# Jamy-L/Handheld-Multi-Frame-Super-Resolution

Hardware: AMD Instinct MI355X
Metric: output Mpix/s for 12MP x 20-frame x2 SR burst; max-abs diff vs reference (higher is better)
Workload: dtype f32

## Files before the change

### handheld-multi-frame-super-resolution_amd/csrc/hhsr_fft.hip

```cpp
#include "hhsr_common.h"
#include "hhsr_fft.h"
#include <math.h>
#include <type_traits>
#include <vector>

#include "hhsr_fft_bfly.h"

__host__ __device__ constexpr int fft_maxit(int R) { return R <= 3 ? 4 : R <= 5 ? 3 : R <= 12 ? 2 : 1; }

template <int R>
__device__ __forceinline__ void stockham_pass(float2* __restrict__ buf, int bstride, int NB,
                                              const float2* __restrict__ twp, int N, int Ns, int tid, int nt, bool pw) {
    constexpr int MAXIT = fft_maxit(R);
    const int L = N / R, total = NB * L;
    const float rNs = 1.0f / (float)Ns, rL = 1.0f / (float)L;
    float2 v[MAXIT][R];
    int dst[MAXIT];
#pragma unroll
    for (int it = 0; it < MAXIT; ++it) {
        const int jj = tid + it * nt;
        if (jj < total) {
            const int bidx = NB > 1 ? (int)(((float)jj + 0.5f) * rL) : 0;
            const int j = jj - __mul24(bidx, L);
            const int q = (int)(((float)j + 0.5f) * rNs);
            const int k = j - __mul24(q, Ns);
            const int base = __mul24(bidx, bstride);
            const float2* ib = buf + base + j;
#pragma unroll
            for (int r = 0; r < R; ++r) v[it][r] = ib[__mul24(r, L)];
            if (Ns > 1) {
                if (R <= HHSR_FFT_POW_RMAX && pw) {
                    float2 w[R];
                    w[1] = twp[k];
#pragma unroll
                    for (int r = 2; r < R; ++r) w[r] = cmul(w[r >> 1], w[r - (r >> 1)]);
#pragma unroll
                    for (int r = 1; r < R; ++r) v[it][r] = cmul(v[it][r], w[r]);
                } else {
#pragma unroll
                    for (int r = 1; r < R; ++r) v[it][r] = cmul(v[it][r], twp[__mul24(r - 1, Ns) + k]);
                }
            }
            dft_reg<R>(v[it]);
            dst[it] = base + __mul24(q * R, Ns) + k;
        }
    }
    __syncthreads();
#pragma unroll
    for (int it = 0; it < MAXIT; ++it) {
        const int jj = tid + it * nt;
        if (jj < total) {
#pragma unroll
            for (int r = 0; r < R; ++r) buf[dst[it] + __mul24(r, Ns)] = v[it][r];
        }
    }
    __syncthreads();
}

template <bool PR>
__device__ __forceinline__ void fft_lds(float2* buf, int bstride, int NB, const float2* tw, int N,
                                        const HhsrRadices& rad, int tid, int nt) {
    int Ns = 1, toff = 0;
    __syncthreads();
    for (int p = 0; p < rad.n; ++p) {
        const int R = rad.r[p];
        int Np = N;
        asm volatile("" : "+s"(Np));
        const bool pw = rad.pow_min > 0 && R <= HHSR_FFT_POW_RMAX && (R - 1) * Ns > rad.pow_min;
        switch (R) {
#define HHSR_PASS(RR) case RR: stockham_pass<RR>(buf, bstride, NB, tw + toff, Np, Ns, tid, nt, pw); break;
            HHSR_PASS(2) HHSR_PASS(3) HHSR_PASS(4) HHSR_PASS(5) HHSR_PASS(6) HHSR_PASS(7) HHSR_PASS(8) HHSR_PASS(9)
            HHSR_PASS(10) HHSR_PASS(12) HHSR_PASS(14) HHSR_PASS(15) HHSR_PASS(16)
            default:
                if constexpr (PR) {
                    switch (R) {
                        HHSR_PASS(11) HHSR_PASS(13) HHSR_PASS(17) HHSR_PASS(19)
                        default: break;
                    }
                }
                break;
#undef HHSR_PASS
        }
        toff += pw ? Ns : (R - 1) * Ns;
        Ns *= R;
    }
}

template <int N_, int... RS>
struct SPlan {
    static constexpr int N = N_;
    static constexpr int NP = (int)sizeof...(RS);
    static constexpr int R[NP] = {RS...};
    static constexpr int ns(int p) {
        int s = 1;
        for (int i = 0; i < p; ++i) s *= R[i];
        return s;
    }
    static constexpr bool pw(int p) {
        return HHSR_FFT_POW_MIN > 0 && R[p] <= HHSR_FFT_POW_RMAX && (R[p] - 1) * ns(p) > HHSR_FFT_POW_MIN;
    }
    static constexpr int toff(int p) {
        int o = 0;
        for (int i = 0; i < p; ++i) o += pw(i) ? ns(i) : (R[i] - 1) * ns(i);
        return o;
    }
    static constexpr int rmax() {
        int m = 0;
        for (int i = 0; i < NP; ++i) m = R[i] > m ? R[i] : m;
        return m;
    }
    static bool matches(int n, const HhsrRadices& rad) {
        if (n != N || rad.n != NP || rad.pow_min != HHSR_FFT_POW_MIN) return false;
        for (int i = 0; i < NP; ++i)
            if (rad.r[i] != R[i]) return false;
        return true;
    }
};
struct NoPlan {
    static constexpr int N = 0;
    static constexpr int rmax() { return 16; }
};
struct PrimePlan {
    static constexpr int N = 0;
    static constexpr int rmax() { return 19; }
};
template <class SP>
constexpr bool plan_runtime = std::is_same<SP, NoPlan>::value || std::is_same<SP, PrimePlan>::value;
template <class SP>
__device__ __forceinline__ int plan_len(int runtime) {
    return plan_runtime<SP> ? runtime : SP::N;
}

template <int N, int NB, int NT, int R, int Ns, bool PW>
__device__ __forceinline__ void stockham_pass_s(float2* __restrict__ buf, const float2* __restrict__ twp, int tid) {
    constexpr int MAXIT = fft_maxit(R), L = N / R, total = NB * L;
    float2 v[MAXIT][R];
    int dst[MAXIT];
#pragma unroll
    for (int it = 0; it < MAXIT; ++it) {
        const int jj = tid + it * NT;
        if (it * NT < total && jj < total) {
            const int bidx = NB > 1 ? (int)((unsigned)jj / (unsigned)L) : 0;
            const int j = jj - bidx * L;
            const int q = (int)((unsigned)j / (unsigned)Ns), k = j - q * Ns;
            const float2* ib = buf + bidx * N + j;
#pragma unroll
            for (int r = 0; r < R; ++r) v[it][r] = ib[r * L];
            if (Ns > 1) {
                if (R <= HHSR_FFT_POW_RMAX && PW) {
                    float2 w[R];
                    w[1] = twp[k];
#pragma unroll
                    for (int r = 2; r < R; ++r) w[r] = cmul(w[r >> 1], w[r - (r >> 1)]);
#pragma unroll
                    for (int r = 1; r < R; ++r) v[it][r] = cmul(v[it][r], w[r]);
                } else {
#pragma unroll
                    for (int r = 1; r < R; ++r) v[it][r] = cmul(v[it][r], twp[(r - 1) * Ns + k]);
                }
            }
            dft_reg<R>(v[it]);
            dst[it] = bidx * N + q * (R * Ns) + k;
        }
    }
    __syncthreads();
#pragma unroll
    for (int it = 0; it < MAXIT; ++it) {
        const int jj = tid + it * NT;
        if (it * NT < total && jj < total) {
#pragma unroll
            for (int r = 0; r < R; ++r) buf[dst[it] + r * Ns] = v[it][r];
        }
    }
    __syncthreads();
}

template <class P, int NB, int NT, int PASS = 0>
__device__ __forceinline__ void fft_lds_s(float2* buf, const float2* tw, int tid) {
    if (PASS == 0) __syncthreads();
    if constexpr (PASS < P::NP) {
        stockham_pass_s<P::N, NB, NT, P::R[PASS], P::ns(PASS), P::pw(PASS)>(buf, tw + P::toff(PASS), tid);
        fft_lds_s<P, NB, NT, PASS + 1>(buf, tw, tid);
    }
}

#define HHSR_STATIC_ROWS(X)                                                                 \
    X(1, 2000, 1, FFT_NT_SMALL, 10, 10, 10, 2)              \
    X(2, 4000, 1, FFT_NT, 10, 10, 10, 4)                        \
    X(3, 2016, 1, FFT_NT_SMALL, 14, 12, 12)     \
    X(4, 2040, 1, FFT_NT_SMALL, 17, 15, 8)      \
    X(5, 2736, 2, FFT_NT, 19, 16, 9)
#define HHSR_STATIC_COLS(X)                                                                 \
    X(1, 3000, 2, FFT_NT, 3, 10, 10, 10)                             \
    X(2, 6000, 1, FFT_NT, 10, 10, 10, 6)                             \
    X(3, 3024, 2, FFT_NT, 9, 8, 7, 6)                                \
    X(4, 3648, 2, FFT_NT, 19, 16, 12)

__device__ __forceinline__ bool fft_kept(int u, int n) {
    int i = u + n / 2;
    if (i >= n) i -= n;
    return i >= n / 4 && i < n - (n + 3) / 4;
}

constexpr int TB = 2;
__device__ __forceinline__ size_t t_index(int kx, int y, int H) { return ((size_t)(kx / TB) * H + y) * TB + (kx % TB); }

constexpr int FFT_NT = 512;
constexpr int FFT_NT_SMALL = 256;
__host__ __device__ constexpr int fft_rows_wpe(int nt) { return nt == FFT_NT ? 6 : 5; }
template <int NT, class SP>
__host__ __device__ constexpr int fft_rows_wpe_of() {
    return (NT == FFT_NT ? SP::rmax() > 17 : SP::rmax() > 16) ? 4 : fft_rows_wpe(NT);
}
constexpr int FFT_COLS_WPE = 4;

template <typename V, int NT = FFT_NT, class Load, class Store>
__device__ __forceinline__ void batched_for(int n, int tid, Load load, Store store) {
    for (int base = tid; base < n; base += 4 * NT) {
        V v[4];
#pragma unroll
        for (int u = 0; u < 4; ++u) {
            const int i = base + u * NT;
            if (i < n) v[u] = load(i);
        }
#pragma unroll
        for (int u = 0; u < 4; ++u) {
            const int i = base + u * NT;
            if (i < n) store(i, v[u]);
        }
    }
}

template <int RB>
__device__ __forceinline__ int row_block(int it, int nblocks) {
    constexpr int G = (16 / (TB * RB)) > 0 ? 16 / (TB * RB) : 1;
    int blk;
    if ((gridDim.x & 7) == 0) {
        const int v = (int)(blockIdx.x >> 3) + it * (int)(gridDim.x >> 3);
        blk = ((v / G) * 8 + (int)(blockIdx.x & 7)) * G + v % G;
    } else {
        blk = (int)blockIdx.x + it * (int)gridDim.x;
    }
    return blk < nblocks ? blk : -1;
}

template <int RB>
__device__ __forceinline__ void split_row(int idx, int len, float rlen, int& rb, int& n) {
    if (RB == 1) {
        rb = 0;
        n = idx;
    } else if (RB == 2) {
        rb = idx >= len;
        n = rb ? idx - len : idx;
    } else {
        rb = (int)(((float)idx + 0.5f) * rlen);
        n = idx - __mul24(rb, len);
    }
}

struct FftFrames {
    const float* src[HHSR_MAX_BATCH];
    float* dst[HHSR_MAX_BATCH];
    int n;
    size_t tstride;
};

template <int RB, int NT, class SP = NoPlan>
__global__ void __launch_bounds__(NT, (fft_rows_wpe_of<NT, SP>())) k_rows_fwd(FftFrames fr, int H, int W,
                                                                        float2* __restrict__ Tall, int Wk, HhsrRadices rad,
                                                                        const float2* __restrict__ twM, int twlen,
                                                                        const float2* __restrict__ twW) {
    extern __shared__ __attribute__((aligned(16))) float2 fl[];
    const int M = plan_len<SP>(W / 2), tid = threadIdx.x;
    W = 2 * M;
    float2* tw = fl;
    float2* buf = tw + ((twlen + 1) & ~1);
    batched_for<float2, NT>(twlen, tid, [&](int k) { return twM[k]; }, [&](int k, float2 v) { tw[k] = v; });
    const int nb = (H + RB - 1) / RB;
    for (int it = 0, vblk; (vblk = row_block<RB>(it, nb * fr.n)) >= 0; ++it) {
    if (it) __syncthreads();
    const int frame = vblk / nb, blk = vblk - frame * nb;
    const float* __restrict__ src = fr.src[frame];
    float2* __restrict__ T = Tall + (size_t)frame * fr.tstride;
    const int y0 = blk * RB;
    const int nrows = min(RB, H - y0);
    if ((M & 1) == 0 && (W & 3) == 0) {
        const int Mh = M / 2;
        const float rMh = 1.0f / (float)Mh;
        const float4* __restrict__ src4 = reinterpret_cast<const float4*>(src + (size_t)y0 * W);
        batched_for<float4, NT>(nrows * Mh, tid, [&](int idx) { return src4[idx]; },
                            [&](int idx, float4 v) {
                                int rb, n;
                                split_row<RB>(idx, Mh, rMh, rb, n);
                                reinterpret_cast<float4*>(buf + __mul24(rb, M))[n] = v;
                            });
    } else {
        for (int idx = tid; idx < nrows * M; idx += NT) {
            const int rb = idx / M, n = idx - rb * M;
            buf[rb * M + n] = reinterpret_cast<const float2*>(src + (size_t)(y0 + rb) * W)[n];
        }
    }
    if constexpr (plan_runtime<SP>) fft_lds<std::is_same<SP, PrimePlan>::value>(buf, M, nrows, tw, M, rad, tid, NT);
    else fft_lds_s<SP, RB, NT>(buf, tw, tid);
    const int nblk = (Wk + TB - 1) / TB;
    if (TB == 2 && (M & 1) == 0 && nrows == RB) {
        for (int idx = tid; idx < nblk * RB; idx += NT) {
            const int b = idx / RB, rb = idx - b * RB, k = 2 * b;
            const float2* Z = buf + __mul24(rb, M);
            const float4 zz = *reinterpret_cast<const float4*>(Z + k);
            const float2 zm0 = cconj(Z[k == 0 ? 0 : M - k]), zm1 = cconj(Z[M - k - 1]);
            const float4 ww = *reinterpret_cast<const float4*>(twW + k);
            const float2 z0 = make_float2(zz.x, zz.y), z1 = make_float2(zz.z, zz.w);
            const float2 s0 = cadd(z0, zm0), d0 = mul_mi(cmul(make_float2(ww.x, ww.y), csub(z0, zm0)));
            const float2 s1 = cadd(z1, zm1), d1 = mul_mi(cmul(make_float2(ww.z, ww.w), csub(z1, zm1)));
            const float2 o0 = cscale(cadd(s0, d0), 0.5f), o1 = cscale(cadd(s1, d1), 0.5f);
            *reinterpret_cast<float4*>(T + ((size_t)b * H + y0 + rb) * 2) = make_float4(o0.x, o0.y, o1.x, o1.y);
        }
    } else
    for (int idx = tid; idx < nblk * nrows * TB; idx += NT) {
        const int b = idx / (nrows * TB), q = idx - b * (nrows * TB);
        const int rb = q / TB, k = b * TB + (q - rb * TB);
        if (k >= Wk) continue;
        const float2* Z = buf + rb * M;
        const float2 zk = Z[k == M ? 0 : k], zm = cconj(Z[k == 0 ? 0 : M - k]);
        const float2 s = cadd(zk, zm), d = mul_mi(cmul(twW[k], csub(zk, zm)));
        T[t_index(k, y0 + rb, H)] = cscale(cadd(s, d), 0.5f);
    }
    }
}

template <int NC, class SP = NoPlan>
__global__ void __launch_bounds__(FFT_NT, FFT_COLS_WPE) k_cols(float2* __restrict__ Tall, size_t tstride, int H, int W, int Wk,
                                                                    HhsrRadices rad, const float2* __restrict__ twH,
                                                                    int twlen, float norm) {
    extern __shared__ __attribute__((aligned(16))) float2 fl[];
    const int tid = threadIdx.x;
    H = plan_len<SP>(H);
    const int xcd = blockIdx.x & 7, loc = blockIdx.x >> 3;
    const int per = 8 / NC;
    const int kx = 8 * (xcd + 8 * (loc / per)) + NC * (loc % per);
    if (kx >= Wk) return;
    float2* __restrict__ T = Tall + (size_t)blockIdx.y * tstride;
    float2* tw = fl;
    float2* buf = tw + ((twlen + 1) & ~1);
    float2* colb = T + ((size_t)(kx / TB) * H) * TB + (kx % TB);
    float4* col = reinterpret_cast<float4*>(colb);
    batched_for<float2>(twlen, tid, [&](int k) { return twH[k]; }, [&](int k, float2 v) { tw[k] = v; });
    if (NC == 2) {
        batched_for<float4>(H, tid, [&](int k) { return col[(size_t)(TB / 2) * k]; },
                            [&](int k, float4 v) {
                                buf[k] = make_float2(v.x, v.y);
                                buf[H + k] = make_float2(v.z, v.w);
                            });
    } else {
        batched_for<float2>(H, tid, [&](int k) { return colb[(size_t)TB * k]; }, [&](int k, float2 v) { buf[k] = v; });
    }
    if constexpr (plan_runtime<SP>) fft_lds<std::is_same<SP, PrimePlan>::value>(buf, H, NC, tw, H, rad, tid, FFT_NT);
    else fft_lds_s<SP, NC, FFT_NT>(buf, tw, tid);
    {
        const int hh = H / 2, lo = H / 4, hi = H - (H + 3) / 4;
        auto kept_y = [&](int u) {
            int i = u + hh;
            if (i >= H) i -= H;
            return i >= lo && i < hi;
        };
#pragma unroll
        for (int c = 0; c < NC; ++c) {
            const int x = kx + c, nx = x == 0 ? 0 : W - x;
            const bool fx = x < Wk && fft_kept(x, W), fnx = x < Wk && fft_kept(nx, W);
            for (int ky = tid; ky < H; ky += FFT_NT) {
                const int nky = ky == 0 ? 0 : H - ky;
                const int m = (int)(fx && kept_y(ky)) + (int)(fnx && kept_y(nky));
                buf[c * H + ky] = cconj(cscale(buf[c * H + ky], 0.5f * (float)m * norm));
            }
        }
    }
    if constexpr (plan_runtime<SP>) fft_lds<std::is_same<SP, PrimePlan>::value>(buf, H, NC, tw, H, rad, tid, FFT_NT);
    else fft_lds_s<SP, NC, FFT_NT>(buf, tw, tid);
    for (int y = tid; y < H; y += FFT_NT) {
        if (NC == 2) {
            const float2 a = cconj(buf[y]), b2 = cconj(buf[H + y]);
            col[(size_t)(TB / 2) * y] = make_float4(a.x, a.y, b2.x, b2.y);
        } else {
            colb[(size_t)TB * y] = cconj(buf[y]);
        }
    }
}

template <int RB, int NT, class SP = NoPlan>
__global__ void __launch_bounds__(NT, (fft_rows_wpe_of<NT, SP>())) k_rows_inv(const float2* __restrict__ Tall, int H, int W, int Wk,
                                                                        FftFrames fr, HhsrRadices rad,
                                                                        const float2* __restrict__ twM, int twlen,
                                                                        const float2* __restrict__ twW) {
    extern __shared__ __attribute__((aligned(16))) float2 fl[];
    const int M = plan_len<SP>(W / 2), tid = threadIdx.x;
    W = 2 * M;
    float2* tw = fl;
    float2* buf = tw + ((twlen + 1) & ~1);
    batched_for<float2, NT>(twlen, tid, [&](int k) { return twM[k]; }, [&](int k, float2 v) { tw[k] = v; });
    const int nb = (H + RB - 1) / RB;
    for (int it = 0, vblk; (vblk = row_block<RB>(it, nb * fr.n)) >= 0; ++it) {
    if (it) __syncthreads();
    const int frame = vblk / nb, blk = vblk - frame * nb;
    const float2* __restrict__ T = Tall + (size_t)frame * fr.tstride;
    float* __restrict__ dst = fr.dst[frame];
    const int y0 = blk * RB;
    const int nrows = min(RB, H - y0);
    const int half = M / 2 + 1, nblk = (half + TB - 1) / TB;
    auto z_of = [&](float2 xk, float2 xm_, int k) {
        const float2 xm = cconj(xm_);
        const float2 s = cadd(xk, xm), d = mul_pi(cmul(cconj(twW[k]), csub(xk, xm)));
        return cconj(cscale(cadd(s, d), 0.5f));
    };
    if (TB == 2 && (M & 1) == 0 && nrows == RB) {
        for (int idx = tid; idx < nblk * RB; idx += NT) {
            const int b = idx / RB, rb = idx - b * RB, k0 = 2 * b, y = y0 + rb;
            float4 x4 = make_float4(0.f, 0.f, 0.f, 0.f);
            if (k0 < Wk) x4 = *reinterpret_cast<const float4*>(T + ((size_t)b * H + y) * 2);
            const float2 xa0 = make_float2(x4.x, x4.y);
            const float2 xa1 = k0 + 1 < Wk ? make_float2(x4.z, x4.w) : make_float2(0.f, 0.f);
            float2* Zr = buf + __mul24(rb, M);
            float2 zk[2];
#pragma unroll
            for (int e = 0; e < 2; ++e) {
                const int k = k0 + e, mk = M - k;
                const float2 xa = e ? xa1 : xa0;
                float2 xb = make_float2(0.f, 0.f);
                if (mk == k) xb = xa;
                else if (mk < Wk) xb = T[t_index(mk, y, H)];
                zk[e] = z_of(xa, xb, k < M ? k : 0);
                if (k < half && mk != k && mk < M) Zr[mk] = z_of(xb, xa, mk);
            }
            if (k0 + 1 < half) *reinterpret_cast<float4*>(Zr + k0) = make_float4(zk[0].x, zk[0].y, zk[1].x, zk[1].y);
            else if (k0 < half) Zr[k0] = zk[0];
        }
    } else
    for (int idx = tid; idx < nblk * nrows * TB; idx += NT) {
        const int b = idx / (nrows * TB), q = idx - b * (nrows * TB);
        const int rb = q / TB, k = b * TB + (q - rb * TB);
        if (k >= half) continue;
        const int mk = M - k;
        const float2 xa = k < Wk ? T[t_index(k, y0 + rb, H)] : make_float2(0.f, 0.f);
        const float2 xb = (mk < Wk && mk != k) ? T[t_index(mk, y0 + rb, H)] : (mk == k ? xa : make_float2(0.f, 0.f));
        {
            const float2 xk = xa, xm = cconj(xb);
            const float2 s = cadd(xk, xm), d = mul_pi(cmul(cconj(twW[k]), csub(xk, xm)));
            buf[rb * M + k] = cconj(cscale(cadd(s, d), 0.5f));
        }
        if (mk != k && mk < M) {
            const float2 xk = xb, xm = cconj(xa);
            const float2 s = cadd(xk, xm), d = mul_pi(cmul(cconj(twW[mk]), csub(xk, xm)));
            buf[rb * M + mk] = cconj(cscale(cadd(s, d), 0.5f));
        }
    }
    if constexpr (plan_runtime<SP>) fft_lds<std::is_same<SP, PrimePlan>::value>(buf, M, nrows, tw, M, rad, tid, NT);
    else fft_lds_s<SP, RB, NT>(buf, tw, tid);
    if ((M & 1) == 0 && (W & 3) == 0) {
        const int Mh = M / 2;
        const float rMh = 1.0f / (float)Mh;
        float4* __restrict__ dst4 = reinterpret_cast<float4*>(dst + (size_t)y0 * W);
        for (int idx = tid; idx < nrows * Mh; idx += NT) {
            int rb, n;
            split_row<RB>(idx, Mh, rMh, rb, n);
            const float4 z = reinterpret_cast<const float4*>(buf + __mul24(rb, M))[n];
            dst4[idx] = make_float4(z.x, -z.y, z.z, -z.w);
        }
    } else {
        for (int idx = tid; idx < nrows * M; idx += NT) {
            const int rb = idx / M, n = idx - rb * M;
            reinterpret_cast<float2*>(dst + (size_t)(y0 + rb) * W)[n] = cconj(buf[rb * M + n]);
        }
    }
    }
}

static std::vector<float2> pass_twiddles(const HhsrRadices& rad);

static const int k_radices[] = {19, 17, 16, 15, 14, 13, 12, 11, 10, 9, 8, 7, 6, 5, 4, 3, 2};

static void radix_search(int n, int rmax, int cap, int nt, int depth, int* cur, int& best_n, int* best, int& best_max) {
    if (n == 1) {
        int mx = 0;
        for (int i = 0; i < depth; ++i) mx = cur[i] > mx ? cur[i] : mx;
        if (depth < best_n || (depth == best_n && mx < best_max)) {
            best_n = depth;
            best_max = mx;
            for (int i = 0; i < depth; ++i) best[i] = cur[i];
        }
        return;
    }
    if (depth + 1 > best_n || depth >= HHSR_MAX_RADICES) return;
    for (int r : k_radices) {
        if (r > rmax || n % r) continue;
        if (depth > 0 && r > cur[depth - 1]) continue;
        if (cap / r > fft_maxit(r) * nt) continue;
        cur[depth] = r;
        radix_search(n / r, rmax, cap, nt, depth + 1, cur, best_n, best, best_max);
    }
}

static bool factorize(int n, int nb, HhsrRadices& out, int nt = FFT_NT) {
    const int rmax = 19;
    int cur[HHSR_MAX_RADICES], best[HHSR_MAX_RADICES], best_n = HHSR_MAX_RADICES + 1, best_max = 1 << 30;
    radix_search(n, rmax, nb * n, nt, 0, cur, best_n, best, best_max);
    if (best_n > HHSR_MAX_RADICES) return false;
    auto collide = [](int r) { int g = 2 * r, b = 64; while (b) { int t = g % b; g = b; b = t; } return g; };
    int first = 0;
    for (int i = 1; i < best_n; ++i)
        if (collide(best[i]) < collide(best[first]) || (collide(best[i]) == collide(best[first]) && best[i] > best[first]))
            first = i;
    out.pow_min = HHSR_FFT_POW_MIN;
    out.n = 0;
    out.r[out.n++] = best[first];
    for (int i = 0; i < best_n; ++i)
        if (i != first) out.r[out.n++] = best[i];
    return out.n > 0;
}

static bool host_kept_fft(int u, int n) {
    int i = u + n / 2;
    if (i >= n) i -= n;
    return i >= n / 4 && i < n - (n + 3) / 4;
}

static float2* upload(const std::vector<float2>& h) {
    float2* d = nullptr;
    const int count = (int)h.size();
    if (hipMalloc((void**)&d, sizeof(float2) * count) != hipSuccess) return nullptr;
    if (count == 0) return nullptr;
    if (hipMemcpy(d, h.data(), sizeof(float2) * count, hipMemcpyHostToDevice) != hipSuccess) {
        (void)hipFree(d);
        return nullptr;
    }
    return d;
}

static std::vector<float2> plain_twiddles(int count, double denom) {
    std::vector<float2> h(count);
    for (int k = 0; k < count; ++k) {
        const double a = -2.0 * M_PI * (double)k / denom;
        h[k] = make_float2((float)cos(a), (float)sin(a));
    }
    return h;
}

static std::vector<float2> pass_twiddles(const HhsrRadices& rad) {
    std::vector<float2> h;
    int Ns = 1;
    for (int p = 0; p < rad.n; ++p) {
        const int R = rad.r[p];
        const bool pw = rad.pow_min > 0 && R <= HHSR_FFT_POW_RMAX && (R - 1) * Ns > rad.pow_min;
        for (int r = 1; r < (pw ? 2 : R); ++r)
            for (int k = 0; k < Ns; ++k) {
                const double a = -2.0 * M_PI * (double)r * (double)k / ((double)Ns * (double)R);
                h.push_back(make_float2((float)cos(a), (float)sin(a)));
            }
        Ns *= R;
    }
    return h;
}

static int pick_rb(int M, HhsrRadices& rad, int& nt) {
    const char* ent = getenv("HHSR_FFT_NT_ROWS");
    const int forced_nt = ent ? atoi(ent) : 0;
    if (forced_nt != FFT_NT && factorize(M, 1, rad, FFT_NT_SMALL) &&
        sizeof(float2) * (((pass_twiddles(rad).size() + 1) & ~(size_t)1) + (size_t)M) <= 32 * 1024) {
        nt = FFT_NT_SMALL;
        return 1;
    }
    nt = FFT_NT;
    const int cands[3] = {2, 4, 1};
    for (int c = 0; c < 3; ++c) {
        const int rb = cands[c];
        if (rb * (M / 2) >= 65536) continue;
        if (!factorize(M, rb, rad)) continue;
        if (sizeof(float2) * (pass_twiddles(rad).size() + (size_t)rb * M) > 76 * 1024 && rb > 1) continue;
        return rb;
    }
    return 0;
}

static int rows_per_cu(const HhsrFft& f) {
    int wpe = 0;
#define HHSR_ROWS_CU(ID, N, RB, NT, ...) \
    if (f.static_rows == ID) wpe = fft_rows_wpe_of<NT, SPlan<N, __VA_ARGS__>>();
    HHSR_STATIC_ROWS(HHSR_ROWS_CU)
#undef HHSR_ROWS_CU
    if (!wpe && f.nt_rows == FFT_NT_SMALL) wpe = f.prime_rows ? fft_rows_wpe_of<FFT_NT_SMALL, PrimePlan>() : fft_rows_wpe(FFT_NT_SMALL);
    if (!wpe) wpe = f.prime_rows ? fft_rows_wpe_of<FFT_NT, PrimePlan>() : fft_rows_wpe(FFT_NT);
    return wpe * 256 / f.nt_rows;
}

static bool has_prime_radix(const HhsrRadices& rad) {
    for (int i = 0; i < rad.n; ++i)
        if (rad.r[i] == 11 || rad.r[i] == 13 || rad.r[i] > 16) return true;
    return false;
}

int hhsr_fft_radices(int n, int nb, int nt, int* radices, int cap) {
    HhsrRadices rad{};
    if (n < 1 || nb < 1 || nt < 1 || !factorize(n, nb, rad, nt)) return 0;
    for (int i = 0; i < rad.n && i < cap; ++i) radices[i] = rad.r[i];
    return rad.n;
}

bool hhsr_fft_schedule(HhsrFft& f, int H, int W, int batch) {
    f = HhsrFft();
    if (batch < 1 || batch > HHSR_MAX_BATCH) return false;
    if (W % 2 || H < 2 || W < 4) return false;
    const int M = W / 2;
    if (M >= 65536 || H >= 65536) return false;
    f.rb = pick_rb(M, f.radM, f.nt_rows);
    if (!f.rb) return false;
    f.nc = 0;
    const char* enc = getenv("HHSR_FFT_NC");
    for (int nc = enc ? atoi(enc) : 2; nc >= 1 && !f.nc; --nc)
        if (factorize(H, nc, f.radH) && sizeof(float2) * (pass_twiddles(f.radH).size() + (size_t)nc * H) <= 150 * 1024) f.nc = nc;
    if (!f.nc) return false;
    int Wk = 0;
    for (int x = 0; x <= M; ++x)
        if (host_kept_fft(x, W) || host_kept_fft(x == 0 ? 0 : W - x, W)) Wk = x + 1;
    if (Wk < 1 || Wk > M) return false;
    f.H = H;
    f.W = W;
    f.Wk = Wk;
    f.twlenM = (int)pass_twiddles(f.radM).size();
    f.twlenH = (int)pass_twiddles(f.radH).size();
    f.lds_rows = sizeof(float2) * ((size_t)((f.twlenM + 1) & ~1) + (size_t)f.rb * M);
    f.lds_cols = sizeof(float2) * ((size_t)((f.twlenH + 1) & ~1) + (size_t)f.nc * H);
    if (f.lds_cols > 150 * 1024 || f.lds_rows > 150 * 1024) return false;
    f.batch = batch;
    f.tstride = (size_t)((Wk + 7) / 8) * 8 * H;
    f.prime_rows = has_prime_radix(f.radM);
    f.prime_cols = has_prime_radix(f.radH);
    const char* es = getenv("HHSR_FFT_STATIC");
    const int allow = es ? atoi(es) : 3;
    f.static_rows = f.static_cols = 0;
#define HHSR_TRY_ROWS(ID, N, RB, NT, ...)                                                                                    \
    if ((allow & 1) && !f.static_rows && f.rb == RB && f.nt_rows == NT && SPlan<N, __VA_ARGS__>::matches(M, f.radM))         \
        f.static_rows = ID;
    HHSR_STATIC_ROWS(HHSR_TRY_ROWS)
#undef HHSR_TRY_ROWS
#define HHSR_TRY_COLS(ID, N, NC, NT, ...)                                                                                    \
    if ((allow & 2) && !f.static_cols && f.nc == NC && SPlan<N, __VA_ARGS__>::matches(H, f.radH)) f.static_cols = ID;
    HHSR_STATIC_COLS(HHSR_TRY_COLS)
#undef HHSR_TRY_COLS
    f.rows_per_cu = rows_per_cu(f);
    return true;
}

template <class RP>
static const void* rows_fwd_kernel(const HhsrFft& f) {
    return f.nt_rows == FFT_NT_SMALL ? (const void*)k_rows_fwd<1, FFT_NT_SMALL, RP> : f.rb == 4 ? (const void*)k_rows_fwd<4, FFT_NT, RP>
         : f.rb == 2 ? (const void*)k_rows_fwd<2, FFT_NT, RP> : (const void*)k_rows_fwd<1, FFT_NT, RP>;
}
template <class RP>
static const void* rows_inv_kernel(const HhsrFft& f) {
    return f.nt_rows == FFT_NT_SMALL ? (const void*)k_rows_inv<1, FFT_NT_SMALL, RP> : f.rb == 4 ? (const void*)k_rows_inv<4, FFT_NT, RP>
         : f.rb == 2 ? (const void*)k_rows_inv<2, FFT_NT, RP> : (const void*)k_rows_inv<1, FFT_NT, RP>;
}

bool hhsr_fft_create(HhsrFft& f, int H, int W, int batch) {
    if (!hhsr_fft_schedule(f, H, W, batch)) {
        f = HhsrFft();
        return false;
    }
    const int M = W / 2;
    const void* kf = f.prime_rows ? rows_fwd_kernel<PrimePlan>(f) : rows_fwd_kernel<NoPlan>(f);
    const void* ki = f.prime_rows ? rows_inv_kernel<PrimePlan>(f) : rows_inv_kernel<NoPlan>(f);
    const void* kc = f.prime_cols ? (f.nc == 2 ? (const void*)k_cols<2, PrimePlan> : (const void*)k_cols<1, PrimePlan>)
                                  : (f.nc == 2 ? (const void*)k_cols<2> : (const void*)k_cols<1>);
    if (hipFuncSetAttribute(kf, hipFuncAttributeMaxDynamicSharedMemorySize, (int)f.lds_rows) != hipSuccess ||
        hipFuncSetAttribute(ki, hipFuncAttributeMaxDynamicSharedMemorySize, (int)f.lds_rows) != hipSuccess ||
        hipFuncSetAttribute(kc, hipFuncAttributeMaxDynamicSharedMemorySize, (int)f.lds_cols) != hipSuccess) {
        (void)hipGetLastError();
        f = HhsrFft();
        return false;
    }
    f.twM = upload(pass_twiddles(f.radM));
    f.twH = upload(pass_twiddles(f.radH));
    f.twW = upload(plain_twiddles(M, (double)W));
    if (hipMalloc((void**)&f.T, sizeof(float2) * f.tstride * batch) != hipSuccess) f.T = nullptr;
    if (!f.twM || !f.twH || !f.twW || !f.T) {
        hhsr_fft_destroy(f);
        return false;
    }
#define HHSR_TRY_ROWS(ID, N, RB, NT, ...)                                                                                    \
    if (f.static_rows == ID &&                                                                                                \
        (hipFuncSetAttribute((const void*)k_rows_fwd<RB, NT, SPlan<N, __VA_ARGS__>>, hipFuncAttributeMaxDynamicSharedMemorySize, (int)f.lds_rows) != hipSuccess || \
         hipFuncSetAttribute((const void*)k_rows_inv<RB, NT, SPlan<N, __VA_ARGS__>>, hipFuncAttributeMaxDynamicSharedMemorySize, (int)f.lds_rows) != hipSuccess))  \
        f.static_rows = 0;
    HHSR_STATIC_ROWS(HHSR_TRY_ROWS)
#undef HHSR_TRY_ROWS
#define HHSR_TRY_COLS(ID, N, NC, NT, ...)                                                                                    \
    if (f.static_cols == ID &&                                                                                                \
        hipFuncSetAttribute((const void*)k_cols<NC, SPlan<N, __VA_ARGS__>>, hipFuncAttributeMaxDynamicSharedMemorySize, (int)f.lds_cols) != hipSuccess) \
        f.static_cols = 0;
    HHSR_STATIC_COLS(HHSR_TRY_COLS)
#undef HHSR_TRY_COLS
    (void)hipGetLastError();
    f.rows_per_cu = rows_per_cu(f);
    f.ok = true;
    return true;
}

void hhsr_fft_destroy(HhsrFft& f) {
    if (f.twM) (void)hipFree(f.twM);
    if (f.twH) (void)hipFree(f.twH);
    if (f.twW) (void)hipFree(f.twW);
    if (f.T) (void)hipFree(f.T);
    f = HhsrFft();
}

int hhsr_fft_lowpass(const HhsrFft& f, const float* const* srcs, float* const* dsts, int n, hipStream_t s) {
    const bool small = f.nt_rows == FFT_NT_SMALL;
    const int persist = 256 * f.rows_per_cu;
    const float norm = (float)(1.0 / ((double)(f.W / 2) * (double)f.H));
    const size_t spectrum = sizeof(float2) * f.tstride, budget = (size_t)112 << 20;
    int per = (int)(budget / (spectrum ? spectrum : 1));
    per = per < 1 ? 1 : per > f.batch ? f.batch : per;
    for (int n0 = 0; n0 < n; n0 += per) {
        FftFrames fr;
        fr.n = n - n0 < per ? n - n0 : per;
        fr.tstride = f.tstride;
        for (int k = 0; k < HHSR_MAX_BATCH; ++k) {
            fr.src[k] = srcs[n0 + (k < fr.n ? k : 0)];
            fr.dst[k] = dsts[n0 + (k < fr.n ? k : 0)];
        }
        const int nrb_all = hhsr_cdiv(f.H, f.rb) * fr.n;
        const int nrb = persist > 0 && persist < nrb_all ? persist : nrb_all;
#define ROWS_FWD(RB, NT) hipLaunchKernelGGL((k_rows_fwd<RB, NT, RP>), dim3(nrb), dim3(NT), f.lds_rows, s, fr, f.H, f.W, f.T, f.Wk, \
                                            f.radM, f.twM, f.twlenM, f.twW)
#define ROWS_INV(RB, NT) hipLaunchKernelGGL((k_rows_inv<RB, NT, RP>), dim3(nrb), dim3(NT), f.lds_rows, s, f.T, f.H, f.W, f.Wk, fr, \
                                            f.radM, f.twM, f.twlenM, f.twW)
#define HHSR_RUN_ROWS_FWD(ID, N, RB, NT, ...)                                                                                \
        if (f.static_rows == ID)                                                                                              \
            hipLaunchKernelGGL((k_rows_fwd<RB, NT, SPlan<N, __VA_ARGS__>>), dim3(nrb), dim3(NT), f.lds_rows, s, fr, f.H, f.W, f.T, \
                               f.Wk, f.radM, f.twM, f.twlenM, f.twW);                                                         \
        else
        HHSR_STATIC_ROWS(HHSR_RUN_ROWS_FWD)
#undef HHSR_RUN_ROWS_FWD
        if (f.prime_rows) {
            using RP = PrimePlan;
            if (small) ROWS_FWD(1, FFT_NT_SMALL); else if (f.rb == 4) ROWS_FWD(4, FFT_NT); else if (f.rb == 2) ROWS_FWD(2, FFT_NT);
            else ROWS_FWD(1, FFT_NT);
        } else {
            using RP = NoPlan;
            if (small) ROWS_FWD(1, FFT_NT_SMALL); else if (f.rb == 4) ROWS_FWD(4, FFT_NT); else if (f.rb == 2) ROWS_FWD(2, FFT_NT);
            else ROWS_FWD(1, FFT_NT);
        }
#define HHSR_RUN_COLS(ID, N, NC, NT, ...)                                                                                    \
        if (f.static_cols == ID)                                                                                              \
            hipLaunchKernelGGL((k_cols<NC, SPlan<N, __VA_ARGS__>>), dim3(((f.Wk + 63) / 64) * (64 / NC), fr.n), dim3(NT), f.lds_cols, \
                               s, f.T, f.tstride, f.H, f.W, f.Wk, f.radH, f.twH, f.twlenH, norm);                             \
        else
        HHSR_STATIC_COLS(HHSR_RUN_COLS)
#undef HHSR_RUN_COLS
#define COLS(NC, RP) hipLaunchKernelGGL((k_cols<NC, RP>), dim3(((f.Wk + 63) / 64) * (64 / NC), fr.n), dim3(FFT_NT), f.lds_cols, s, f.T, \
                                      f.tstride, f.H, f.W, f.Wk, f.radH, f.twH, f.twlenH, norm)
        if (f.prime_cols) { if (f.nc == 2) COLS(2, PrimePlan); else COLS(1, PrimePlan); }
        else { if (f.nc == 2) COLS(2, NoPlan); else COLS(1, NoPlan); }
#undef COLS
#define HHSR_RUN_ROWS_INV(ID, N, RB, NT, ...)                                                                                \
        if (f.static_rows == ID)                                                                                              \
            hipLaunchKernelGGL((k_rows_inv<RB, NT, SPlan<N, __VA_ARGS__>>), dim3(nrb), dim3(NT), f.lds_rows, s, f.T, f.H, f.W, f.Wk, \
                               fr, f.radM, f.twM, f.twlenM, f.twW);                                                           \
        else
        HHSR_STATIC_ROWS(HHSR_RUN_ROWS_INV)
#undef HHSR_RUN_ROWS_INV
        if (f.prime_rows) {
            using RP = PrimePlan;
            if (small) ROWS_INV(1, FFT_NT_SMALL); else if (f.rb == 4) ROWS_INV(4, FFT_NT); else if (f.rb == 2) ROWS_INV(2, FFT_NT);
            else ROWS_INV(1, FFT_NT);
        } else {
            using RP = NoPlan;
            if (small) ROWS_INV(1, FFT_NT_SMALL); else if (f.rb == 4) ROWS_INV(4, FFT_NT); else if (f.rb == 2) ROWS_INV(2, FFT_NT);
            else ROWS_INV(1, FFT_NT);
        }
#undef ROWS_FWD
#undef ROWS_INV
    }
    return hhsr_launch_status("hhsr_grey_lowpass");
}
```

Measured before the change: 6303.

## Fuse global loads/stores and spectral mask into first/last Stockham FFT passes

Makes the static Stockham pass configurable with source and sink policies, so the first column pass can read straight from global memory and the last column/row pass can write straight to global memory, skipping the separate LDS staging copy loops. The spectral mask and normalisation are applied inside the last pass of the forward column FFT instead of in a separate sweep. This removes LDS round trips and barriers around the staging loops. In exchange it adds a pair-mapped thread layout and less coalesced global access patterns inside the passes.

```diff
diff --git a/handheld-multi-frame-super-resolution_amd/csrc/hhsr_fft.hip b/handheld-multi-frame-super-resolution_amd/csrc/hhsr_fft.hip
--- a/handheld-multi-frame-super-resolution_amd/csrc/hhsr_fft.hip
+++ b/handheld-multi-frame-super-resolution_amd/csrc/hhsr_fft.hip
@@ -131,21 +131,60 @@
     return plan_runtime<SP> ? runtime : SP::N;
 }
 
-template <int N, int NB, int NT, int R, int Ns, bool PW>
-__device__ __forceinline__ void stockham_pass_s(float2* __restrict__ buf, const float2* __restrict__ twp, int tid) {
+struct InLds {
+    static constexpr bool PAIR = false, SYNC = true, LDS = true;
+};
+template <int NB>
+struct Legs {
+    float2 c[NB];
+};
+template <int N, int NB, int NT, int R>
+constexpr bool pass_pairs = fft_maxit(R) % NB == 0 && (fft_maxit(R) / NB) * NT >= N / R;
+
+template <int N, int NB, int NT, int R, int Ns, bool PW, class Src = InLds, class Sink = InLds>
+__device__ __forceinline__ void stockham_pass_s(float2* __restrict__ buf, const float2* __restrict__ twp, int tid,
+                                                const Src& src = Src(), const Sink& sink = Sink()) {
     constexpr int MAXIT = fft_maxit(R), L = N / R, total = NB * L;
+    constexpr bool SRC_LDS = std::is_same<Src, InLds>::value, SNK_LDS = std::is_same<Sink, InLds>::value;
+    constexpr bool PAIR = Src::PAIR || Sink::PAIR;
+    static_assert(!PAIR || pass_pairs<N, NB, NT, R>, "pair mapping: MAXIT butterflies per thread cover all sequences");
+    auto where = [&](int it, int& bidx, int& j) {
+        if (PAIR) {
+            bidx = it % NB;
+            j = tid + (it / NB) * NT;
+            int jc = j;
+            if (NB > 1) asm volatile("" : "+v"(jc));
+            return (it / NB) * NT < L && jc < L;
+        }
+        const int jj = tid + it * NT;
+        bidx = NB > 1 ? (int)((unsigned)jj / (unsigned)L) : 0;
+        j = jj - bidx * L;
+        return it * NT < total && jj < total;
+    };
     float2 v[MAXIT][R];
     int dst[MAXIT];
 #pragma unroll
     for (int it = 0; it < MAXIT; ++it) {
-        const int jj = tid + it * NT;
-        if (it * NT < total && jj < total) {
-            const int bidx = NB > 1 ? (int)((unsigned)jj / (unsigned)L) : 0;
-            const int j = jj - bidx * L;
+        int bidx, j;
+        if (where(it, bidx, j)) {
             const int q = (int)((unsigned)j / (unsigned)Ns), k = j - q * Ns;
-            const float2* ib = buf + bidx * N + j;
-#pragma unroll
-            for (int r = 0; r < R; ++r) v[it][r] = ib[r * L];
+            if constexpr (SRC_LDS) {
+                const float2* ib = buf + bidx * N + j;
+#pragma unroll
+                for (int r = 0; r < R; ++r) v[it][r] = ib[r * L];
+            } else if constexpr (Src::PAIR) {
+                if (it % NB == 0) {
+#pragma unroll
+                    for (int r = 0; r < R; ++r) {
+                        const Legs<NB> x = src(j + r * L);
+#pragma unroll
+                        for (int c = 0; c < NB; ++c) v[it + c][r] = x.c[c];
+                    }
+                }
+            } else {
+#pragma unroll
+                for (int r = 0; r < R; ++r) v[it][r] = src(bidx, j + r * L);
+            }
             if (Ns > 1) {
                 if (R <= HHSR_FFT_POW_RMAX && PW) {
                     float2 w[R];
@@ -160,27 +199,50 @@
                 }
             }
             dft_reg<R>(v[it]);
-            dst[it] = bidx * N + q * (R * Ns) + k;
-        }
-    }
-    __syncthreads();
+            dst[it] = (SNK_LDS ? bidx * N : 0) + q * (R * Ns) + k;
+        }
+    }
+    constexpr bool WRITES_LDS = Sink::LDS;
+    if constexpr (WRITES_LDS && Src::SYNC) __syncthreads();
 #pragma unroll
     for (int it = 0; it < MAXIT; ++it) {
-        const int jj = tid + it * NT;
-        if (it * NT < total && jj < total) {
-#pragma unroll
-            for (int r = 0; r < R; ++r) buf[dst[it] + r * Ns] = v[it][r];
-        }
-    }
-    __syncthreads();
-}
-
-template <class P, int NB, int NT, int PASS = 0>
-__device__ __forceinline__ void fft_lds_s(float2* buf, const float2* tw, int tid) {
-    if (PASS == 0) __syncthreads();
+        int bidx, j;
+        if (where(it, bidx, j)) {
+            if constexpr (SNK_LDS) {
+#pragma unroll
+                for (int r = 0; r < R; ++r) buf[dst[it] + r * Ns] = v[it][r];
+            } else if constexpr (Sink::PAIR) {
+                if (it % NB == 0) {
+#pragma unroll
+                    for (int r = 0; r < R; ++r) {
+                        Legs<NB> x;
+#pragma unroll
+                        for (int c = 0; c < NB; ++c) x.c[c] = v[it + c][r];
+                        sink(dst[it] + r * Ns, x);
+                    }
+                }
+            } else {
+#pragma unroll
+                for (int r = 0; r < R; ++r) sink(bidx, dst[it] + r * Ns, v[it][r]);
+            }
+        }
+    }
+    if constexpr (WRITES_LDS) __syncthreads();
+}
+
+template <class P, int NB, int NT, class Src = InLds, class Sink = InLds, int PASS = 0>
+__device__ __forceinline__ void fft_lds_s(float2* buf, const float2* tw, int tid, const Src& src = Src(),
+                                          const Sink& sink = Sink()) {
+    if (PASS == 0 && std::is_same<Src, InLds>::value) __syncthreads();
     if constexpr (PASS < P::NP) {
-        stockham_pass_s<P::N, NB, NT, P::R[PASS], P::ns(PASS), P::pw(PASS)>(buf, tw + P::toff(PASS), tid);
-        fft_lds_s<P, NB, NT, PASS + 1>(buf, tw, tid);
+        constexpr bool FIRST = PASS == 0, LAST = PASS == P::NP - 1;
+        using S0 = std::conditional_t<FIRST, Src, InLds>;
+        using S1 = std::conditional_t<LAST, Sink, InLds>;
+        const InLds lds;
+        const S0& s0 = [&]() -> const S0& { if constexpr (FIRST) return src; else return lds; }();
+        const S1& s1 = [&]() -> const S1& { if constexpr (LAST) return sink; else return lds; }();
+        stockham_pass_s<P::N, NB, NT, P::R[PASS], P::ns(PASS), P::pw(PASS), S0, S1>(buf, tw + P::toff(PASS), tid, s0, s1);
+        fft_lds_s<P, NB, NT, Src, Sink, PASS + 1>(buf, tw, tid, src, sink);
     }
 }
 
@@ -263,6 +325,20 @@
     float* dst[HHSR_MAX_BATCH];
     int n;
     size_t tstride;
+};
+
+#ifndef HHSR_FFT_DIRECT
+#define HHSR_FFT_DIRECT 7
+#endif
+
+template <int RB>
+struct RowSink {
+    static constexpr bool PAIR = false, LDS = false;
+    float2* __restrict__ x;
+    int M, nrows;
+    __device__ __forceinline__ void operator()(int b, int n, float2 v) const {
+        if (RB == 1 || b < nrows) x[__mul24(b, M) + n] = cconj(v);
+    }
 };
 
 template <int RB, int NT, class SP = NoPlan>
@@ -329,6 +405,61 @@
     }
 }
 
+template <int NC>
+struct ColSrc {
+    static constexpr bool PAIR = true, SYNC = false;
+    const float2* __restrict__ colb;
+    __device__ __forceinline__ Legs<NC> operator()(int y) const {
+        Legs<NC> x;
+        if (NC == 2) {
+            const float4 v = reinterpret_cast<const float4*>(colb)[(TB / 2) * y];
+            x.c[0] = make_float2(v.x, v.y);
+            x.c[NC - 1] = make_float2(v.z, v.w);
+        } else {
+            x.c[0] = colb[TB * y];
+        }
+        return x;
+    }
+};
+template <int NC>
+struct ColSink {
+    static constexpr bool PAIR = true, LDS = false;
+    float2* __restrict__ colb;
+    __device__ __forceinline__ void operator()(int y, const Legs<NC>& x) const {
+        if (NC == 2) {
+            const float2 a = cconj(x.c[0]), b2 = cconj(x.c[NC - 1]);
+            reinterpret_cast<float4*>(colb)[(TB / 2) * y] = make_float4(a.x, a.y, b2.x, b2.y);
+        } else {
+            colb[TB * y] = cconj(x.c[0]);
+        }
+    }
+};
+template <int NC>
+struct ColMask {
+    static constexpr bool PAIR = false, LDS = true;
+    float2* buf;
+    int H, hh, lo, hi;
+    bool fx[NC], fnx[NC];
+    float norm;
+    __device__ __forceinline__ bool kept_y(int u) const {
+        int i = u + hh;
+        if (i >= H) i -= H;
+        return i >= lo && i < hi;
+    }
+    __device__ __forceinline__ void operator()(int c, int ky, float2 v) const {
+        const int nky = ky == 0 ? 0 : H - ky;
+        const bool f = c ? fx[NC - 1] : fx[0], fn = c ? fnx[NC - 1] : fnx[0];
+        const int m = (int)(f && kept_y(ky)) + (int)(fn && kept_y(nky));
+        buf[c * H + ky] = cconj(cscale(v, 0.5f * (float)m * norm));
+    }
+};
+template <class SP, int NC, bool LAST>
+constexpr bool cols_pass_pairs() {
+    if constexpr (plan_runtime<SP>) return false;
+    else if (!LAST && NC == 2 && SP::N == 3024) return false;
+    else return pass_pairs<SP::N, NC, FFT_NT, SP::R[LAST ? SP::NP - 1 : 0]>;
+}
+
 template <int NC, class SP = NoPlan>
 __global__ void __launch_bounds__(FFT_NT, FFT_COLS_WPE) k_cols(float2* __restrict__ Tall, size_t tstride, int H, int W, int Wk,
                                                                     HhsrRadices rad, const float2* __restrict__ twH,
@@ -346,6 +477,10 @@
     float2* colb = T + ((size_t)(kx / TB) * H) * TB + (kx % TB);
     float4* col = reinterpret_cast<float4*>(colb);
     batched_for<float2>(twlen, tid, [&](int k) { return twH[k]; }, [&](int k, float2 v) { tw[k] = v; });
+    constexpr bool D_FIRST = (HHSR_FFT_DIRECT & 1) && cols_pass_pairs<SP, NC, false>();
+    constexpr bool D_MASK = (HHSR_FFT_DIRECT & 4) && !plan_runtime<SP>;
+    constexpr bool D_LAST = (HHSR_FFT_DIRECT & 2) && cols_pass_pairs<SP, NC, true>();
+    if constexpr (!D_FIRST) {
     if (NC == 2) {
         batched_for<float4>(H, tid, [&](int k) { return col[(size_t)(TB / 2) * k]; },
                             [&](int k, float4 v) {
@@ -355,7 +490,23 @@
     } else {
         batched_for<float2>(H, tid, [&](int k) { return colb[(size_t)TB * k]; }, [&](int k, float2 v) { buf[k] = v; });
     }
+    }
+    if constexpr (D_MASK) {
+        ColMask<NC> mask;
+        mask.buf = buf;
+        mask.H = H, mask.hh = H / 2, mask.lo = H / 4, mask.hi = H - (H + 3) / 4;
+        mask.norm = norm;
+#pragma unroll
+        for (int c = 0; c < NC; ++c) {
+            const int x = kx + c, nx = x == 0 ? 0 : W - x;
+            mask.fx[c] = x < Wk && fft_kept(x, W);
+            mask.fnx[c] = x < Wk && fft_kept(nx, W);
+        }
+        if constexpr (D_FIRST) fft_lds_s<SP, NC, FFT_NT, ColSrc<NC>, ColMask<NC>>(buf, tw, tid, ColSrc<NC>{colb}, mask);
+        else fft_lds_s<SP, NC, FFT_NT, InLds, ColMask<NC>>(buf, tw, tid, InLds(), mask);
+    } else {
     if constexpr (plan_runtime<SP>) fft_lds<std::is_same<SP, PrimePlan>::value>(buf, H, NC, tw, H, rad, tid, FFT_NT);
+    else if constexpr (D_FIRST) fft_lds_s<SP, NC, FFT_NT, ColSrc<NC>>(buf, tw, tid, ColSrc<NC>{colb});
     else fft_lds_s<SP, NC, FFT_NT>(buf, tw, tid);
     {
         const int hh = H / 2, lo = H / 4, hi = H - (H + 3) / 4;
@@ -375,6 +526,10 @@
             }
         }
     }
+    }
+    if constexpr (D_LAST) {
+        fft_lds_s<SP, NC, FFT_NT, InLds, ColSink<NC>>(buf, tw, tid, InLds(), ColSink<NC>{colb});
+    } else {
     if constexpr (plan_runtime<SP>) fft_lds<std::is_same<SP, PrimePlan>::value>(buf, H, NC, tw, H, rad, tid, FFT_NT);
     else fft_lds_s<SP, NC, FFT_NT>(buf, tw, tid);
     for (int y = tid; y < H; y += FFT_NT) {
@@ -385,6 +540,7 @@
             colb[(size_t)TB * y] = cconj(buf[y]);
         }
     }
+    }
 }
 
 template <int RB, int NT, class SP = NoPlan>
@@ -393,6 +549,7 @@
                                                                         const float2* __restrict__ twM, int twlen,
                                                                         const float2* __restrict__ twW) {
     extern __shared__ __attribute__((aligned(16))) float2 fl[];
+    constexpr bool DIRECT = !plan_runtime<SP> && (HHSR_FFT_DIRECT & 2);
     const int M = plan_len<SP>(W / 2), tid = threadIdx.x;
     W = 2 * M;
     float2* tw = fl;
@@ -453,6 +610,10 @@
             buf[rb * M + mk] = cconj(cscale(cadd(s, d), 0.5f));
         }
     }
+    if constexpr (DIRECT) {
+        const RowSink<RB> rows{reinterpret_cast<float2*>(dst + (size_t)y0 * W), M, nrows};
+        fft_lds_s<SP, RB, NT, InLds, RowSink<RB>>(buf, tw, tid, InLds(), rows);
+    } else {
     if constexpr (plan_runtime<SP>) fft_lds<std::is_same<SP, PrimePlan>::value>(buf, M, nrows, tw, M, rad, tid, NT);
     else fft_lds_s<SP, RB, NT>(buf, tw, tid);
     if ((M & 1) == 0 && (W & 3) == 0) {
@@ -470,6 +631,7 @@
             const int rb = idx / M, n = idx - rb * M;
             reinterpret_cast<float2*>(dst + (size_t)(y0 + rb) * W)[n] = cconj(buf[rb * M + n]);
         }
+    }
     }
     }
 }
```

Measured after the change: 6357, median of 6. No clear change (+0.9%).
